# fanzhongyi/diffusion

Measured on AMD Instinct MI355X. Metric: U-Net training images/sec @256 (SD-2-base U-Net, precomputed latents 4x32x32), higher is better.
Workload: dtype bf16; 1 GPU; SD-2-base U-Net train step, latents 4x32x32, text 77x1024, batch 256/GPU (global 256), microbatch 256, AdamW, dp1; global_batch=256, microbatch=256, parallelism=dp1, params=865910724

## Files before the change

diffusion_amd/_lib.py:

```python
from __future__ import annotations

import ctypes as C
import os

_HERE = os.path.dirname(os.path.abspath(__file__))
LIB_PATH = os.path.join(_HERE, os.environ.get('DA_LIB_ALT') or 'libdiffusion_amd.so')

_vp, _l, _i, _f, _fp, _ll = C.c_void_p, C.c_long, C.c_int, C.c_float, C.c_void_p, C.c_void_p



class DaWgradItem(C.Structure):
    _fields_ = [('dY', C.c_void_p), ('lddy', C.c_long), ('X', C.c_void_p), ('ldx', C.c_long), ('dW', C.c_void_p),
                ('dbias', C.c_void_p), ('N', C.c_int), ('Cin', C.c_int)]


SIGNATURES = {
    'da_gemm_nt': [_vp, _l, _vp, _vp, _l, _fp, _vp, _l, _vp, _l, _i, _i, _i, _i, _i, _i, _i, _i, _i, _i, _i, _f, _fp, _l,
                   _vp],
    'da_set_option': [C.c_char_p, _i],
    'da_gemm_nt_variant_for': [_i, _i, _i, _i, _l],
    'da_gemm_nt_geglu': [_vp, _l, _vp, _vp, _l, _vp, _l, _fp, _i, _i, _i, _vp],
    'da_gemm_nt_geglu_bwd': [_vp, _l, _vp, _vp, _l, _vp, _l, _i, _i, _i, _vp],
    'da_gemm_tn_wgrad': [_vp, _l, _vp, _l, _fp, _fp, _fp, _i, _i, _i, _i, _i, _i, _i, _i, _i, _fp, _l, _vp],
    'da_gemm_tn_variant_for': [_i, _i, _i, _i, _i, _i, _i, _i, _i],
    'da_gemm_tn_wgrad_group': [C.POINTER(DaWgradItem), _i, _i, _fp, _l, _vp],
    'da_gemm_tn_group_plan': [C.POINTER(DaWgradItem), _i, _i, _l, C.POINTER(_i), _i, C.POINTER(_i)],
    'da_attn_fwd': [_vp, _l, _vp, _l, _vp, _l, _vp, _l, _fp, _i, _i, _i, _i, _f, _vp],
    'da_attn_fwd_causal': [_vp, _l, _vp, _l, _vp, _l, _vp, _l, _fp, _i, _i, _i, _f, _vp],
    'da_attn_fwd_wide': [_vp, _l, _vp, _l, _vp, _l, _vp, _l, _fp, _i, _i, _i, _i, _i, _f, _vp],
    'da_attn_bwd': [_vp, _l, _vp, _l, _vp, _l, _vp, _l, _vp, _l, _fp, _fp, _vp, _l, _vp, _l, _vp, _l, _i, _i, _i, _i,
                    _f, _vp],
    'da_norm_scratch_floats': [_i, _i, _i],
    'da_groupnorm_fwd': [_vp, _l, _vp, _l, _fp, _fp, _fp, _fp, _fp, _i, _i, _i, _i, _f, _i, _vp],
# ... 87 lines not shown
```

diffusion_amd/csrc/gemm_nt.hip:

```cpp
#include <string.h>

#include "common.hpp"
#include "diffusion_amd.h"

namespace {

struct GemmNTParams {
  const bf16* A;
  const bf16* W;
  void* C;
  const float* bias;
  const bf16* rowbias;
  const bf16* R;
  long lda, ldc, ldrb, ldr;
  int M, N, K, Cin;
  int Hin, Win, Hout, Wout;
  int ksize, mode;
  int out_fp32;
  float alpha;
  int tiles_m, tiles_n;
};

constexpr int BM = 128, BN = 128, BK = 64;
constexpr int STAGE_BYTES = (BM + BN) * BK * 2;
// ... 203 lines not shown
                           hipStream_t stream);

int da_gemm_nt_v3_try(const void* A, long lda, const void* W, void* C, long ldc, const float* bias, const void* R, long ldr,
                      int M, int N, int K, hipStream_t stream);
extern int g_nt_stream, g_nt_stream_lw;
int da_gemm_nt_ws_try(const void* A, long lda, const void* W, const float* bias, const void* R, long ldr, void* C, long ldc,
                      int M, int N, int K, hipStream_t stream);
extern int g_nt_ws;

extern int g_tn_variant;
extern int g_nt_korder;
extern int g_nt_persist;
extern int g_reserve_cus;
extern int g_nt_persist_conv;
extern int g_nt_de;
extern int g_grad_overwrite;
extern int g_attn_fused_bwd;
extern int g_tn_ring, g_tn_ungroup;
extern int g_gn_resident, g_gn_resident_form, g_gn_resident_min_slab;
int da_usable_cus(int cus);
static int g_nt_variant = 0;
static int g_nt_mfma32 = 0;
static int g_nt_splitk = 1;

static int g_nt_dispatch = 1;

static int pick_nt_variant_legacy(int M, int N, int K, int Cin, long ws_floats, int* splits) {
  *splits = 1;
  const long tm = (M + 255) / 256;
  if (N % 320 == 0 && tm * (N / 320) >= 160) return 12;
// ... 102 lines not shown
    return DA_OK;
  }
  if (key && !strcmp(key, "gemm_nt_stream_lw")) {
    if (value != 4 && value != 16) return DA_ERR_SHAPE;
    g_nt_stream_lw = value;
    return DA_OK;
  }
  if (key && !strcmp(key, "gemm_nt_stream")) {
    g_nt_stream = value;
    return DA_OK;
  }
  if (key && !strcmp(key, "gemm_nt_de")) {
    g_nt_de = value;
    return DA_OK;
  }
  if (key && !strcmp(key, "gemm_nt_persist_conv")) {
    g_nt_persist_conv = value;
    return DA_OK;
  }
  if (key && !strcmp(key, "gn_resident")) {
    if (value < 0) return DA_ERR_SHAPE;
    g_gn_resident = value;
    return DA_OK;
  }
  if (key && !strcmp(key, "gn_resident_min_slab")) {
    if (value < 0) return DA_ERR_SHAPE;
    g_gn_resident_min_slab = value;
    return DA_OK;
  }
  if (key && !strcmp(key, "gn_resident_form")) {
// ... 62 lines not shown
```

diffusion_amd/csrc/gemm_nt_v2.hip:

```cpp
#include "common.hpp"
#include "diffusion_amd.h"
#ifndef NT2_NT
#define NT2_NT 0
#endif
#if NT2_NT
#define NTST st8_nt
#else
#define NTST st8
#endif


#ifndef NT2_CT
#define NT2_CT 1
#endif

int g_nt_persist = -1;
int g_reserve_cus = 0;
int g_nt_persist_conv = 1;
int g_nt_de = 1;
int da_usable_cus(int cus) {
  int n = cus - g_reserve_cus;
  return n < 32 ? 32 : n;
}

// ... 12 lines not shown
  int ksize, mode;
  int out_fp32;
  float alpha;
  int tiles_m, tiles_n;
  int splits, ksteps_per_split;
  long slab_stride;
  bf16* G;
  long ldg;
  int inner;
  int total_blocks;
  FastDiv div_hw, div_w;
  FastDiv div_nblk, div_tn;
  int korder;
};

__device__ __attribute__((aligned(256))) unsigned char g_zero_page[256];

template <int BK>
DEVINL int swz_key(int row) { return BK == 64 ? ((row >> 1) & 7) : ((row >> 2) & 3); }
template <int BK>
DEVINL int swz2(int row, int chunk) { return row * (BK * 2) + ((chunk ^ swz_key<BK>(row)) << 4); }

DEVINL void lds_barrier() {
  asm volatile("s_waitcnt lgkmcnt(0)" ::: "memory");
  __builtin_amdgcn_s_barrier();
  asm volatile("" ::: "memory");
}

#ifdef DA_STAMPS
__device__ unsigned long long* g_stamp_buf;
// ... 2 lines not shown
    if (threadIdx.x == 0 && g_stamp_buf) g_stamp_buf[(long)vblock * 16 + (i)] = __builtin_amdgcn_s_memtime(); \
  } while (0)
extern "C" int da_debug_set_stamps(void* buf) {
  return hipMemcpyToSymbol(HIP_SYMBOL(g_stamp_buf), &buf, sizeof(buf)) == hipSuccess ? 0 : -1;
}
#else
#define STAMP(i) do {} while (0)
#endif

DEVINL void glds16(const void* gsrc, char* lds_dst) {
  __builtin_amdgcn_global_load_lds((const __attribute__((address_space(1))) void*)gsrc,
                                   (__attribute__((address_space(3))) void*)lds_dst, 16, 0, 0);
}

template <int MT, int NT, int WM, int WN, int BK, bool UPS, int GEGLU, bool EARLY, int MF = 16, bool PERSIST = EARLY, bool DE = false,
          bool HASR = false>
DEVINL void nt2_tile(const GemmNT2Params& p, const int vblock0, char* smem) {
  constexpr int NW = WM * WN;
  constexpr bool CT = MF == 16 && GEGLU == 0 && ((NT2_CT && !EARLY) || DE);
  static_assert(!DE || (MF == 16 && GEGLU == 0 && ((NT % 2) == 0 || (MT % 2) == 0)), "direct epilogue: 16x16 tiles in pairs");
  constexpr int V2_BM = MF * MT * WM, V2_BK = BK;
  static_assert((NW == 16 || NW == 8 || NW == 4) && (BK == 64 || BK == 32), "wave grid");
  static_assert(MF == 16 || (MF == 32 && GEGLU == 0 && BK == 64), "MFMA shape");
  constexpr int BN = MF * NT * WN;
  constexpr int SR = MF == 16 ? 16 : 8;
  constexpr int RG = 512 / BK;
  constexpr int LR = BK / 8;
  constexpr int AJ = V2_BM / RG / NW;
  constexpr int BGROUPS = BN / RG;
  constexpr int BJ = (BGROUPS + NW - 1) / NW;
  constexpr int A_BYTES = V2_BM * V2_BK * 2;
  constexpr int B_BYTES = BN * V2_BK * 2;
// ... 11 lines not shown
  auto task_of = [&](int ln, int pss, int tasks) {
    const bool ragged_last = (tasks % (64 * WN)) != 0 && pss == (tasks + 64 * WN - 1) / (64 * WN) - 1;
    const int slot = ragged_last ? (wn + WN - (wm * WN / 4) % WN) % WN : wn;
    return slot * 64 + ln + 64 * WN * pss;
  };
  auto fresh_lane = [&]() {
    int ln = lane;
    asm volatile("" : "+v"(ln));
    return ln;
  };
  STAMP(0);

  const int nblk = p.tiles_m * p.tiles_n;
  int split, tn, m0, n0;
  auto locate = [&](int vb) {
    split = (PERSIST && !EARLY) ? (int)fdiv((unsigned)vb, p.div_nblk) : vb / nblk;
    int bid = vb - split * nblk;
    const int q = nblk >> 3, r = nblk & 7;
    const int xcd = bid & 7, idx = bid >> 3;
    bid = (xcd < r ? xcd * (q + 1) : r * (q + 1) + (xcd - r) * q) + idx;
    const int tm = (PERSIST && !EARLY) ? (int)fdiv((unsigned)bid, p.div_tn) : bid / p.tiles_n;
    tn = bid - tm * p.tiles_n;
    m0 = tm * V2_BM;
    n0 = tn * BN;
  };
  auto wrow = [&](int c) {
    if constexpr (GEGLU == 1) return c < BN / 2 ? tn * (BN / 2) + c : p.inner + tn * (BN / 2) + (c - BN / 2);
    else return n0 + c;
  };
  const int HWo = p.Hout * p.Wout;
  constexpr bool PCONV = PERSIST && !EARLY;
  const int pad = PCONV ? 1 : ((p.ksize == 3 && p.mode != 4) ? 1 : 0);
  const int gmul = PCONV ? 1 : ((p.mode == 1 || p.mode == 4) ? 2 : 1), gshift = PCONV ? 0 : ((p.mode == 2 || p.mode == 3) ? 1 : 0),
            pmask = PCONV ? 0 : ((p.mode == 2) ? 1 : 0);
  const int hlim = gshift ? 2 * p.Hin : p.Hin, wlim = gshift ? 2 * p.Win : p.Win;
  const char* zero = reinterpret_cast<const char*>(g_zero_page);
  auto load_bias = [&](int buf) {
    if (tid < BN / 4) {
      const int n = wrow(tid * 4);
      const void* src = (p.bias && n < p.N) ? (const void*)(p.bias + n) : (const void*)zero;
      glds16(src, smem + BIAS_OFF + buf * (BN * 4) + wave * 1024);
    }
  };

  const int ntaps = PCONV ? 9 : p.ksize * p.ksize;
  const bf16* abase[AJ];
  unsigned amask[AJ];
  unsigned aoff[AJ];
  unsigned woff[BJ];
  int nk, tap, c0;
  const int nk_total = p.K / V2_BK;
  const bool tap_inner = p.korder != 0 && ntaps > 1;
  auto describe = [&]() {
  const int dl = fresh_lane();
  const int lrow = dl / LR, lchunk = dl % LR;
#pragma unroll
// ... 30 lines not shown
    }
    const int bh = (oh * gmul - pad) >> gshift, bw = (ow * gmul - pad) >> gshift;
    if constexpr (PERSIST && !UPS) {
      aoff[j] = (unsigned)(((long)(b * p.Hin * p.Win) + (long)bh * p.Win + bw) * p.lda * 2 + (lchunk ^ swz_key<BK>(row)) * 16);
      if (j == 0) amask[0] = mask & 0x1ffu;
      else amask[0] |= (mask & 0x1ffu) << (9 * j);
      continue;
    }
    amask[j] = mask;
    abase[j] = p.A + ((long)(b * p.Hin * p.Win) + (long)bh * p.Win + bw) * p.lda + (lchunk ^ swz_key<BK>(row)) * 8;
  }
#pragma unroll
  for (int j = 0; j < BJ; ++j) {
    const int g = wave + NW * j;
    const int row = g * RG + lrow;
    const int n = min(wrow(row), p.N - 1);
    woff[j] = ((unsigned)n * (unsigned)p.K + (lchunk ^ swz_key<BK>(row)) * 8) * 2;
  }

  const int kstep_begin = split * p.ksteps_per_split;
  nk = min(p.ksteps_per_split, nk_total - kstep_begin);
  if (tap_inner) {
    const int ch = kstep_begin / ntaps;
    tap = kstep_begin - ch * ntaps;
    c0 = ch * V2_BK;
  } else {
    const int kb = kstep_begin * V2_BK;
    tap = kb / p.Cin;
    c0 = kb - tap * p.Cin;
  }
  };
  auto issue = [&](int stage, bool live) {
// ... 22 lines not shown
        for (int j = 0; j < AJ; ++j) {
          const void* src = (amask[j] & tapbit) ? (const void*)(abase[j] + soff) : (const void*)zero;
          glds16(src, Ab + (wave * AJ + j) * 1024);
        }
      }
    } else {
#pragma unroll
      for (int j = 0; j < AJ; ++j) {
        const int ph = (amask[j] >> 16) & 1, pw = (amask[j] >> 17) & 1;
        const int dr = (r + pad * (1 - ph)) >> 1, ds = (s2 + pad * (1 - pw)) >> 1;
        const long soff = (long)(dr * p.Win + ds) * p.lda + c0;
        const void* src = (amask[j] & tapbit) ? (const void*)(abase[j] + soff) : (const void*)zero;
        glds16(src, Ab + (wave * AJ + j) * 1024);
      }
    }
    const char* wb = reinterpret_cast<const char*>(p.W + (live ? tap * p.Cin + c0 : 0));
#pragma unroll
    for (int j = 0; j < BJ; ++j) {
      const int g = wave + NW * j;
      if constexpr (PERSIST && !EARLY) {
        if (BGROUPS % NW == 0 || g < BGROUPS) glds16(wb + (size_t)j * (NW * RG) * p.K * 2 + woff[0], Bb + g * 1024);
      } else {
        if (BGROUPS % NW == 0 || g < BGROUPS) glds16(wb + woff[j], Bb + g * 1024);
      }
    }
    const int tap_n = tap + 1, c_n = c0 + V2_BK;
    const bool wrap_t = tap_n >= ntaps, wrap_c = c_n >= p.Cin;
    if (tap_inner) {
      tap = wrap_t ? 0 : tap_n;
      c0 = wrap_t ? c_n : c0;
    } else {
// ... 317 lines not shown

  constexpr bool EPI_DB = !PERSIST && 2 * WM * STRIP * 4 <= 2 * STAGE;
  constexpr int CH = BN / 8;
  constexpr int TASKS = SR * CH;
  constexpr int NSI = MT * (MF == 16 ? 1 : 4);
  constexpr int PASSES = (TASKS + 64 * WN - 1) / (64 * WN);
  constexpr int RBUD = NW == 16 ? 3 : 10;
  constexpr int RD = (NSI < RBUD / PASSES) ? NSI : (RBUD / PASSES < 1 ? 1 : RBUD / PASSES);
  int trow[PASSES], tcol[PASSES];
  bool tval[PASSES];
#pragma unroll
  for (int pss = 0; pss < PASSES; ++pss) {
    const int task = task_of(el, pss, TASKS);
    trow[pss] = task / CH;
    tcol[pss] = (task - trow[pss] * CH) * 8;
    tval[pss] = task < TASKS && n0e + tcol[pss] < p.N;
  }
  const int mrow0 = m0e + wm * (MF * MT);
  const bool has_r = p.R != nullptr && p.splits == 1;
  bf16x8 rres[RD][PASSES];
  auto fetch_r = [&](int i, int slot) {
#pragma unroll
    for (int pss = 0; pss < PASSES; ++pss) {
      const int m = mrow0 + i * SR + trow[pss];
      if (tval[pss] && m < p.M) rres[slot][pss] = ld8(p.R + (long)m * p.ldr + n0e + tcol[pss]);
    }
  };
#pragma unroll
  for (int i = 0; i < RD; ++i) {
#pragma unroll
// ... 53 lines not shown
          for (int e = 0; e < 8; ++e) v[e] += bf2f(rbv[e]);
        }
        if (has_r) {
          const bf16x8 rv = rres[i % RD][pss];
#pragma unroll
          for (int e = 0; e < 8; ++e) v[e] += bf2f(rv[e]);
        }
        if (p.out_fp32) {
          float* cp = reinterpret_cast<float*>(p.C) + (long)m * p.ldc + n;
          *reinterpret_cast<f32x4*>(cp) = f32x4{v[0], v[1], v[2], v[3]};
          *reinterpret_cast<f32x4*>(cp + 4) = f32x4{v[4], v[5], v[6], v[7]};
        } else {
          bf16x8 o;
#pragma unroll
          for (int e = 0; e < 8; ++e) o[e] = f2bf(v[e]);
          if constexpr (EARLY) NTST(reinterpret_cast<bf16*>(p.C) + (long)m * p.ldc + n, o);
          else st8(reinterpret_cast<bf16*>(p.C) + (long)m * p.ldc + n, o);
        }
      }
    }
    if (has_r && i + RD < NSI) fetch_r(i + RD, i % RD);
    if (!EPI_DB) lds_barrier();
    STAMP(4 + i);
  }
  };

  locate(vblock);
  load_bias(0);
  describe();
  issue(0, true);
  if constexpr (!PERSIST) {
    kloop(0);
    epilogue(m0, n0, tn, split, 0);
  } else {
    for (int bbuf = 0;; bbuf ^= 1) {
      kloop(bbuf);
      const int m0e = m0, n0e = n0, tne = tn, splite = split;
      const int vnext = vblock + (int)gridDim.x;
      const bool more = vnext < p.total_blocks;
      if (more) {
        locate(vnext);
        load_bias(bbuf ^ 1);
        describe();
        issue(0, true);
      }
      STAMP(8);
      epilogue(m0e, n0e, tne, splite, bbuf);
      STAMP(12);
      if (!more) break;
      vblock = vnext;
    }
  }
}

template <int MT, int NT, int WM, int WN, int BK, bool UPS, int GEGLU = 0, bool EARLY = false, int MF = 16, bool PERSIST = EARLY, bool DE = false,
          bool HASR = false>
__global__ __launch_bounds__(64 * WM * WN, (WM * WN == 16 ? 4 : 2)) void gemm_nt2_kernel(GemmNT2Params p) {
  extern __shared__ __attribute__((aligned(16))) char smem[];
  nt2_tile<MT, NT, WM, WN, BK, UPS, GEGLU, EARLY, MF, PERSIST, DE, HASR>(p, blockIdx.x, smem);
}

__global__ void splitk_finalize_kernel(GemmNT2Params p, const float* ws) {
  const int nvec = p.N >> 3;
  const long total = (long)p.M * nvec;
  const int HWo = p.Hout * p.Wout;
  for (long i = (long)blockIdx.x * blockDim.x + threadIdx.x; i < total; i += (long)gridDim.x * blockDim.x) {
    const long m = i / nvec;
    const int n = (int)(i - m * nvec) * 8;
    float v[8] = {0.f, 0.f, 0.f, 0.f, 0.f, 0.f, 0.f, 0.f};
#pragma unroll 4
    for (int s = 0; s < p.splits; ++s) {
      const float* src = ws + s * p.slab_stride + m * p.N + n;
      const f32x4 a = *reinterpret_cast<const f32x4*>(src), b = *reinterpret_cast<const f32x4*>(src + 4);
#pragma unroll
// ... 129 lines not shown
    if (p.ksize == 1 && (long)p.M * p.lda * 2 < (1L << 32)) return launch_v2_mode<MT, NT, WM, WN, BK, false, true, MF>(p, splits, ws, stream);
  }
  if constexpr (WM * WN == 16 && MF == 16 && MT == 4 && NT == 5) {
    const long tiles = (long)((p.M + 255) / 256) * ((p.N + 319) / 320) * (splits > 1 ? splits : 1);
    if (g_nt_persist_conv && g_nt_persist != 0 && p.ksize == 3 && p.mode == 0 && tiles > da_usable_cus(256) && p.N % 320 == 0 &&
        p.M < (1 << 24) && (long)p.M * p.Hout * p.Wout < (1L << 40) &&
        (long)(p.M / (p.Hout * p.Wout)) * p.Hin * p.Win * p.lda * 2 < (1L << 32))
      return launch_v2_mode<MT, NT, WM, WN, BK, false, false, MF, true>(p, splits, ws, stream);
  }
  return launch_v2_mode<MT, NT, WM, WN, BK, false, false, MF>(p, splits, ws, stream);
}

}

int g_nt_korder = 1;

int da_gemm_nt_v2_dispatch(int variant, int splits, float* ws, const void* A, long lda, const void* W, void* C, long ldc, const float* bias,
                           const void* rowbias, long ldrb, const void* R, long ldr, int M, int N, int K, int Cin,
                           int Hin, int Win, int Hout, int Wout, int ksize, int mode, int out_fp32, float alpha,
                           hipStream_t stream) {
  GemmNT2Params p;
  p.A = (const bf16*)A; p.W = (const bf16*)W; p.C = C; p.bias = bias;
  p.rowbias = (const bf16*)rowbias; p.R = (const bf16*)R;
  p.lda = lda; p.ldc = ldc; p.ldrb = ldrb; p.ldr = ldr;
  p.M = M; p.N = N; p.K = K; p.Cin = Cin;
  p.Hin = Hin; p.Win = Win; p.Hout = Hout; p.Wout = Wout;
  p.ksize = ksize; p.mode = mode; p.out_fp32 = out_fp32; p.alpha = alpha;
  p.tiles_m = p.tiles_n = 0;
  p.splits = 1; p.ksteps_per_split = 0; p.slab_stride = 0;
  p.G = nullptr; p.ldg = 0; p.inner = 0;
// ... 62 lines not shown
```

diffusion_amd/models/unet.py:

```python
from __future__ import annotations

import math
import os
from dataclasses import dataclass
from typing import Dict, List, Optional, Tuple

import torch
import torch.nn as nn

from .. import ops
from ..ops import BF16, F32, Geom


@dataclass
class UNetConfig:
    in_channels: int = 4
    out_channels: int = 4
    block_out_channels: Tuple[int, ...] = (320, 640, 1280, 1280)
    attention_head_dim: Tuple[int, ...] = (5, 10, 20, 20)
    cross_attention_dim: int = 1024
    layers_per_block: int = 2
    norm_num_groups: int = 32
    norm_eps: float = 1e-5
    sample_size: int = 64
# ... 286 lines not shown
        self.exp_avg_sq = torch.zeros(fp.total, device=dev, dtype=F32)
        self.shadow = torch.zeros(fp.total, device=dev, dtype=BF16)
        self.shadow_t = torch.zeros(max(fp.total_t, 8), device=dev, dtype=BF16)
        self._bind_views()
        self._scratch = None
        self._scratch_key = None
        self.opt_step = 0
        self._grad_fresh = False
        self._grad_ready_cb = None
        import os
        self.wgrad_stream = torch.cuda.Stream() if os.environ.get('DA_WGRAD_STREAM', '0') == '1' else None
        self._wgrad_defer = None
        self._tape = None
        self._kv, self._record = None, True
        self._ctx = self._tproj = None
        if init:
            self.reset_parameters(seed)

    def _bind_views(self):
        fp = self.fp
        self._mats: Dict[str, Mat] = {}
        self._vecs: Dict[str, Vec] = {}
        for name, st in fp.storages.items():
            sl = slice(st.off, st.off + st.numel)
            if st.ntc is not None:
                N, T, C = st.ntc
                m = Mat()
                m.N, m.T, m.C = N, T, C
                m.w = self.shadow[sl].view(N, T * C)
                m.gw = self.grad[sl].view(N, T * C)
# ... 266 lines not shown
        tb = p + '.transformer_blocks.0'
        g, gst = self._gn_fwd(x, p + '.norm', B, HW, 1e-6, 0)
        h0 = self._lin_fwd(g, p + '.proj_in')
        n1, ln1 = self._ln_fwd(h0, tb + '.norm1')
        qkv = self._bf(M, 3 * C)
        ops.gemm_nt(n1, self.M(tb + '.attn1.qkv.weight').w, qkv, Geom.linear(M))
        o1 = self._bf(M, C)
        l1 = self._f32(B * heads * HW)
        ops.attn_fwd(qkv[:, :C], qkv[:, C:2 * C], qkv[:, 2 * C:], o1, l1, B, heads, HW, HW, 0.125)
        h1 = self._lin_fwd(o1, tb + '.attn1.to_out.0', residual=h0)
        n2, ln2 = self._ln_fwd(h1, tb + '.norm2')
        q2 = self._lin_fwd(n2, tb + '.attn2.to_q', bias=False)
        nk = self._ctx.shape[0] // B
        if self._kv is not None:
            kv2 = self._kv[p]
        else:
            kv2 = self._bf(B * nk, 2 * C)
            ops.gemm_nt(self._ctx, self.M(tb + '.attn2.kv.weight').w, kv2, Geom.linear(B * nk))
        o2 = self._bf(M, C)
        l2 = self._f32(B * heads * HW)
        ops.attn_fwd(q2, kv2[:, :C], kv2[:, C:], o2, l2, B, heads, HW, nk, 0.125)
        h2 = self._lin_fwd(o2, tb + '.attn2.to_out.0', residual=h1)
        n3, ln3 = self._ln_fwd(h2, tb + '.norm3')
        gg = self._bf(M, 4 * C)
        if ops.geglu_fusable(4 * C, C):
            f = self._bf(M, 8 * C)
            ops.gemm_nt_geglu(n3, self.M(tb + '.ff.net.0.proj.weight').w, f, gg, self.V(tb + '.ff.net.0.proj.bias').p)
        else:
            f = self._lin_fwd(n3, tb + '.ff.net.0.proj')
            ops.geglu_fwd(f, gg)
# ... 26 lines not shown
        if ops.geglu_bwd_fusable(4 * C, C):
            self._lin_bwd(gg, dh3, tb + '.ff.net.2', need_dx=False)
            ops.gemm_nt_geglu_bwd(dh3, self.M(tb + '.ff.net.2.weight').wt, f, df)
        else:
            dgg = self._lin_bwd(gg, dh3, tb + '.ff.net.2')
            ops.geglu_bwd(f, dgg, df)
            del dgg
        dn3 = self._lin_bwd(n3, df, tb + '.ff.net.0.proj')
        del df
        dh2 = self._ln_bwd(h2, dn3, dh3, tb + '.norm3', ln3)
        do2 = self._lin_bwd(o2, dh2, tb + '.attn2.to_out.0')
        dq2 = self._bf(M, C)
        dkv2 = self._bf(B * nk, 2 * C)
        ops.attn_bwd(q2, kv2[:, :C], kv2[:, C:], o2, do2, l2, self._delta, dq2, dkv2[:, :C], dkv2[:, C:], B, heads, HW,
                     nk, 0.125)
        self._wgrad(dkv2, self._ctx, self.M(tb + '.attn2.kv.weight').gw, Geom.linear(B * nk))
        dn2 = self._lin_bwd(n2, dq2, tb + '.attn2.to_q', bias=False)
        dh1 = self._ln_bwd(h1, dn2, dh2, tb + '.norm2', ln2)
        do1 = self._lin_bwd(o1, dh1, tb + '.attn1.to_out.0')
        dqkv = self._bf(M, 3 * C)
        ops.attn_bwd(qkv[:, :C], qkv[:, C:2 * C], qkv[:, 2 * C:], o1, do1, l1, self._delta, dqkv[:, :C],
                     dqkv[:, C:2 * C], dqkv[:, 2 * C:], B, heads, HW, HW, 0.125)
        mq = self.M(tb + '.attn1.qkv.weight')
        self._wgrad(dqkv, n1, mq.gw, Geom.linear(M))
        dn1 = self._bf(M, C)
        ops.gemm_nt(dqkv, mq.wt, dn1, Geom.linear(M))
        dh0 = self._ln_bwd(h0, dn1, dh1, tb + '.norm1', ln1)
        dg = self._lin_bwd(g, dh0, p + '.proj_in')
        if self._wgrad_defer is not None:
            items, self._wgrad_defer = self._wgrad_defer[1], None
            ops.gemm_tn_wgrad_group(items, M)
# ... 3 lines not shown
    def forward_features(self, xt8: torch.Tensor, t: torch.Tensor, ctx: torch.Tensor, B: int, S, kv=None,
                         record: bool = True):
        if kv is None and record:
            return self._walk(xt8, t, ctx, B, S)
        if kv is not None and record:
            raise ValueError('forward_features: kv is for the forward-only walk (backward needs the projections it made)')
        keep = (self._ctx, self._tproj)
        self._kv, self._record = kv, False
        try:
            return self._walk(xt8, t, ctx, B, S)
        finally:
            self._kv, self._record = None, True
            self._ctx, self._tproj = keep

    def project_context(self, ctx: torch.Tensor):
        kv = {}
        for key in self._mats:
            if key.endswith('.attn2.kv.weight'):
                m = self.M(key)
                out = self._bf(ctx.shape[0], m.N)
                ops.gemm_nt(ctx, m.w, out, Geom.linear(ctx.shape[0]))
                kv[key[:-len('.transformer_blocks.0.attn2.kv.weight')]] = out
        return kv

    def _walk(self, xt8, t, ctx, B, S):
        cfg = self.cfg
        boc = cfg.block_out_channels
        n = len(boc)
        record = self._record
        H, W = spatial_hw(S)
        self.check_spatial(H, W)
        if xt8.shape[0] != B * H * W:
            raise ValueError(f'forward_features: {xt8.shape[0]} input rows for B * H * W = {B} * {H} * {W}')
        self._ensure_scratch(B, H, W)
        self._ctx = ctx
        tape = [] if record else _NoTape()
        te0 = self._bf(B, boc[0])
        if t.dtype == F32:
            ops.timestep_embed_f32(t, te0)
        else:
            ops.timestep_embed(t, te0)
        te1 = self._lin_fwd(te0, 'time_embedding.linear_1')
        te1s = self._bf(B, cfg.time_embed_dim)
        ops.silu_fwd(te1, te1s)
        temb = self._lin_fwd(te1s, 'time_embedding.linear_2')
        tembs = self._bf(B, cfg.time_embed_dim)
        ops.silu_fwd(temb, tembs)
        self._tproj = self._bf(B, self.tproj_total)
        ops.gemm_nt(tembs, self.M('time_emb_proj_all.weight').w, self._tproj, Geom.linear(B),
                    bias=self.V('time_emb_proj_all.bias').p)
# ... 65 lines not shown
                    tape.append(('resnet', sv))
                    h, sv = self._transformer_fwd(f'up_blocks.{i}.attentions.{j}', h, B, rh, rw, rev_heads[i], out=nxt)
                    tape.append(('transformer', sv))
                else:
                    h, sv = self._resnet_fwd(p, cat, B, rh, rw, out=nxt)
                    tape.append(('resnet', sv))
                if not record:
                    cats[s] = cat = None
                s -= 1
            if i < n - 1:
                key = f'up_blocks.{i}.upsamplers.0.conv'
                y = cats[s][:, :cat_cb[s]]
                ops.gemm_nt(h, self.M(key + '.weight').w, y, Geom.up(B, rh, rw), bias=self.V(key + '.bias').p)
                tape.append(('up', (key, h, B, rh, rw)))
                h = y
        a, st = self._gn_fwd(h, 'conv_norm_out', B, H * W, cfg.norm_eps, 1)
        pred = torch.empty(B * H * W, 8, device=self.device_, dtype=F32)
        ops.gemm_nt(a, self.M('conv_out.weight').w, pred, Geom.conv(B, H, W), bias=self.V('conv_out.bias').p)
        if not record:
            return pred
        tape.append(('out', (h, a, st, B, H, W)))
        self._tape = tape
        self._cats = cats
        return pred

    def backward_features(self, dpred: torch.Tensor):
        tape, self._tape = self._tape, None
        if tape is None:
            raise RuntimeError('backward_features called without a recorded forward')
        fresh, self._grad_fresh = getattr(self, '_grad_fresh', False), False
        if fresh:
            ops.set_option('grad_overwrite', 1)
        try:
            self._backward_walk(tape, dpred)
        finally:
            if fresh:
                ops.set_option('grad_overwrite', 0)

    def _backward_walk(self, tape, dpred: torch.Tensor):
        B = dpred.shape[0]
        self._dtproj = self._bf(self._tproj.shape[0], self.tproj_total)
        dskip: Dict[int, torch.Tensor] = {}
        dh = None
        off = lambda name: self.fp.storages[name].off
        for kind, sv in reversed(tape):
            lo = None
            if kind == 'out':
                lo = off('conv_norm_out.weight')
                h, a, st, B, H, W = sv
                m = self.M('conv_out.weight')
                g3 = Geom.conv(B, H, W)
                self._wgrad(dpred, a, m.gw, g3, dbias=self.V('conv_out.bias').g, scratch=self._scratch)
                da = self._bf(B * H * W, m.C)
                ops.gemm_nt(dpred, m.wt, da, g3)
                dh = self._gn_bwd(h, da, None, 'conv_norm_out', st, B, H * W, 1)
            elif kind == 'resnet':
                dh = self._resnet_bwd(sv, dh)
                lo = off(sv[0] + '.norm1.weight')
            elif kind == 'transformer':
# ... 27 lines not shown
                ops.gemm_nt(dh, m.wt, dx, Geom.down_dgrad(B, rh, rw))
                dh = dx
            elif kind == 'conv_in':
                xt8, B, H, W = sv
                tot = self._bf(*dh.shape)
                ops.add(dh, dskip.pop(0), tot)
                self._wgrad(tot, xt8, self.M('conv_in.weight').gw, Geom.conv(B, H, W),
                                  dbias=self.V('conv_in.bias').g, scratch=self._scratch)
                lo = off('conv_in.weight')
            else:
                raise AssertionError(kind)
            if lo is not None and self._grad_ready_cb is not None:
                if self.wgrad_stream is not None:
                    torch.cuda.current_stream().wait_stream(self.wgrad_stream)
                self._grad_ready_cb(lo)
        te0, te1, te1s, temb, tembs = self._temb_saved
        Bt = te0.shape[0]
        mt = self.M('time_emb_proj_all.weight')
        self._wgrad(self._dtproj, tembs, mt.gw, Geom.linear(Bt), dbias=self.V('time_emb_proj_all.bias').g,
                          scratch=self._scratch)
        dtembs = self._bf(Bt, mt.C)
        ops.gemm_nt(self._dtproj, mt.wt, dtembs, Geom.linear(Bt))
        dtemb = self._bf(Bt, mt.C)
        ops.silu_bwd(temb, dtembs, dtemb)
        dte1s = self._lin_bwd(te1s, dtemb, 'time_embedding.linear_2')
        dte1 = self._bf(*te1.shape)
        ops.silu_bwd(te1, dte1s, dte1)
        self._lin_bwd(te0, dte1, 'time_embedding.linear_1', need_dx=False)
        if self.wgrad_stream is not None:
            torch.cuda.current_stream().wait_stream(self.wgrad_stream)
# ... 32 lines not shown
```

diffusion_amd/ops.py:

```python
from __future__ import annotations

import ctypes
import os
from typing import Optional, Tuple

import torch

from . import _lib

BF16 = torch.bfloat16
F32 = torch.float32


def _stream() -> int:
    return torch.cuda.current_stream().cuda_stream


SPLITK_WS = None


PROFILE = None


class _Timed:
# ... 122 lines not shown
                14: 'gemm_nt2_kernel<4,4,4,4>', 15: 'gemm_nt2_kernel<1,5,8,2,mf32>', 16: 'gemm_nt2_kernel<2,5,4,2,mf32>',
                18: 'gemm_nt2_kernel<3,4,8,2>'}[v]
        ws = _opt('gemm_nt_ws', 1)
        ws_bn = 320 if (K == 320 and (ws & 1) and N <= 1280) else 128 if (K == 640 and (ws & 2) and N <= 1024) else 0
        if (ws_bn and _opt('gemm_nt_variant', 0) == 0 and N % ws_bn == 0 and M % 32 == 0 and (M // 32) * (N // ws_bn) >= 8 * 256
                and g.ksize == 1 and g.mode == 0 and not out_fp32 and alpha == 1.0 and rowbias is None):
            name = 'gemm_nt_ws_kernel'
    with _Timed(name, flops, (M, N, K, g.ksize, g.mode)):
        _lib.call('da_gemm_nt', a_ptr, lda, w_ptr, c_ptr, ldc, _vec(bias, N, 'bias'), rb_ptr, ldrb, r_ptr, ldr, M, N,
                  K, Cin, g.Hin, g.Win, g.Hout, g.Wout, g.ksize, g.mode, int(out_fp32), float(alpha),
                  SPLITK_WS.data_ptr() if SPLITK_WS is not None else 0,
                  SPLITK_WS.numel() if SPLITK_WS is not None else 0, _stream())
    return out


def geglu_fusable(inner: int, K: int) -> bool:
    return inner % 160 == 0 and K % 64 == 0


def gemm_nt_geglu(A, W, F, G, bias):
    a_ptr, lda = _mat(A, BF16, 'A')
    w_ptr, ldw = _mat(W, BF16, 'W')
    f_ptr, ldf = _mat(F, BF16, 'F')
    g_ptr, ldg = _mat(G, BF16, 'G')
    M, K = A.shape
    inner = G.shape[1]
    if tuple(W.shape) != (2 * inner, K) or ldw != K or tuple(F.shape) != (M, 2 * inner) or G.shape[0] != M:
        raise ValueError('gemm_nt_geglu: shape mismatch')
    if not geglu_fusable(inner, K):
        raise ValueError(f'gemm_nt_geglu needs inner % 160 == 0 and K % 64 == 0, got {inner}, {K}')
# ... 660 lines not shown
```

include/diffusion_amd.h:

```cpp
#ifndef DIFFUSION_AMD_H
#define DIFFUSION_AMD_H

#ifdef __cplusplus
extern "C" {
#endif

typedef struct ihipStream_t* da_stream_t;

int da_gemm_nt(const void* A, long lda, const void* W, void* C, long ldc, const float* bias, const void* rowbias,
               long ldrb, const void* R, long ldr, int M, int N, int K, int Cin, int Hin, int Win, int Hout, int Wout,
               int ksize, int mode, int out_fp32, float alpha, float* splitk_ws, long splitk_ws_floats,
               da_stream_t stream);

int da_gemm_nt_geglu(const void* A, long lda, const void* W, void* F, long ldf, void* G, long ldg, const float* bias,
                     int M, int inner, int K, da_stream_t stream);

int da_gemm_nt_geglu_bwd(const void* dY, long lddy, const void* Wt, const void* F, long ldf, void* dF, long lddf, int M,
                         int inner, int K, da_stream_t stream);

int da_set_option(const char* key, int value);
int da_gemm_nt_variant_for(int M, int N, int K, int Cin, long splitk_ws_floats);

int da_gemm_tn_wgrad(const void* dY, long lddy, const void* X, long ldx, float* dW, float* dbias, float* scratch, int M,
                     int N, int Cin, int Hin, int Win, int Hout, int Wout, int ksize, int mode, float* split_ws,
                     long split_ws_floats, da_stream_t stream);

int da_gemm_tn_variant_for(int M, int N, int Cin, int Hin, int Win, int Hout, int Wout, int ksize, int mode);

typedef struct DaWgradItem {
  const void* dY;
  long lddy;
  const void* X;
  long ldx;
// ... 148 lines not shown
```

Before: 1586 images/sec.

## Group cross-attention KV projections into one persistent GEMM and batch their wgrads

Adds a grouped persistent GEMM kernel that computes every cross-attention KV projection of the shared text context in a single launch (up to 16 weight matrices). Tiles are walked in patches across the concatenated N dimension. The forward pass precomputes all KV projections up front, and the backward pass defers the KV weight-gradient GEMMs into one grouped wgrad call at the end. This cuts many small launches and under-filled GEMMs on the 77-token context. The cost is holding all KV outputs live across the whole forward pass, plus a new, complex tile-mapping code path.

```diff
diff --git a/diffusion_amd/_lib.py b/diffusion_amd/_lib.py
--- a/diffusion_amd/_lib.py
+++ b/diffusion_amd/_lib.py
@@ -15,9 +15,16 @@
                 ('dbias', C.c_void_p), ('N', C.c_int), ('Cin', C.c_int)]
 
 
+class DaGemmNtItem(C.Structure):
+    _fields_ = [('W', C.c_void_p), ('C', C.c_void_p), ('ldc', C.c_long), ('bias', C.c_void_p), ('N', C.c_int),
+                ('reserved', C.c_int)]
+
+
 SIGNATURES = {
     'da_gemm_nt': [_vp, _l, _vp, _vp, _l, _fp, _vp, _l, _vp, _l, _i, _i, _i, _i, _i, _i, _i, _i, _i, _i, _i, _f, _fp, _l,
                    _vp],
+    'da_gemm_nt_group': [_vp, _l, C.POINTER(DaGemmNtItem), _i, _i, _i, _vp],
+    'da_gemm_nt_group_plan': [C.POINTER(DaGemmNtItem), _i, _i, _i],
     'da_set_option': [C.c_char_p, _i],
     'da_gemm_nt_variant_for': [_i, _i, _i, _i, _l],
     'da_gemm_nt_geglu': [_vp, _l, _vp, _vp, _l, _vp, _l, _fp, _i, _i, _i, _vp],
diff --git a/diffusion_amd/csrc/gemm_nt.hip b/diffusion_amd/csrc/gemm_nt.hip
--- a/diffusion_amd/csrc/gemm_nt.hip
+++ b/diffusion_amd/csrc/gemm_nt.hip
@@ -241,6 +241,7 @@
 extern int g_reserve_cus;
 extern int g_nt_persist_conv;
 extern int g_nt_de;
+extern int g_kv_group, g_nt_group_patch;
 extern int g_grad_overwrite;
 extern int g_attn_fused_bwd;
 extern int g_tn_ring, g_tn_ungroup;
@@ -373,6 +374,16 @@
     g_nt_de = value;
     return DA_OK;
   }
+  if (key && !strcmp(key, "kv_group")) {
+    if (value != 0 && value != 1) return DA_ERR_SHAPE;
+    g_kv_group = value;
+    return DA_OK;
+  }
+  if (key && !strcmp(key, "gemm_nt_group_patch")) {
+    if (value < 0 || value > 9999) return DA_ERR_SHAPE;
+    g_nt_group_patch = value;
+    return DA_OK;
+  }
   if (key && !strcmp(key, "gemm_nt_persist_conv")) {
     g_nt_persist_conv = value;
     return DA_OK;
diff --git a/diffusion_amd/csrc/gemm_nt_v2.hip b/diffusion_amd/csrc/gemm_nt_v2.hip
--- a/diffusion_amd/csrc/gemm_nt_v2.hip
+++ b/diffusion_amd/csrc/gemm_nt_v2.hip
@@ -50,6 +50,27 @@
   int korder;
 };
 
+constexpr int NT_GROUP_MAX = 16;
+struct NtGroupItem {
+  const bf16* W;
+  bf16* C;
+  const float* bias;
+  long ldc;
+  int N;
+  int first;
+};
+struct NtGroupParams {
+  NtGroupItem it[NT_GROUP_MAX];
+  int patch_m, patch_n;
+};
+
+struct NtGroupState {
+  int item, eitem;
+  const bf16* W;
+  const float* bias;
+  int N;
+};
+
 __device__ __attribute__((aligned(256))) unsigned char g_zero_page[256];
 
 template <int BK>
@@ -82,8 +103,9 @@
 }
 
 template <int MT, int NT, int WM, int WN, int BK, bool UPS, int GEGLU, bool EARLY, int MF = 16, bool PERSIST = EARLY, bool DE = false,
-          bool HASR = false>
-DEVINL void nt2_tile(const GemmNT2Params& p, const int vblock0, char* smem) {
+          bool HASR = false, bool GROUP = false>
+DEVINL void nt2_tile(const GemmNT2Params& p, const int vblock0, char* smem, const NtGroupParams* gp = nullptr, NtGroupState* gs = nullptr) {
+  static_assert(!GROUP || (EARLY && PERSIST && GEGLU == 0 && !DE && !HASR && !UPS && MF == 16), "grouped form: persistent linear tile walk");
   constexpr int NW = WM * WN;
   constexpr bool CT = MF == 16 && GEGLU == 0 && ((NT2_CT && !EARLY) || DE);
   static_assert(!DE || (MF == 16 && GEGLU == 0 && ((NT % 2) == 0 || (MT % 2) == 0)), "direct epilogue: 16x16 tiles in pairs");
@@ -125,6 +147,34 @@
   const int nblk = p.tiles_m * p.tiles_n;
   int split, tn, m0, n0;
   auto locate = [&](int vb) {
+    if constexpr (GROUP) {
+      const int nb = p.tiles_m * p.tiles_n;
+      const int q = nb >> 3, r = nb & 7;
+      const int xcd = vb & 7, idx = vb >> 3;
+      const int bid = (xcd < r ? xcd * (q + 1) : r * (q + 1) + (xcd - r) * q) + idx;
+      const int band_tiles = p.tiles_m * gp->patch_n;
+      const int cb = min(bid / band_tiles, (p.tiles_n - 1) / gp->patch_n);
+      const int bb = bid - cb * band_tiles;
+      const int w = min(gp->patch_n, p.tiles_n - cb * gp->patch_n);
+      const int pt = gp->patch_m * w;
+      const int rp = bb / pt, rem = bb - rp * pt;
+      const int pr = rem / w;
+      const int tm = rp * gp->patch_m + pr, tc = cb * gp->patch_n + (rem - pr * w);
+      int it = 0;
+#pragma unroll
+      for (int i = 1; i < NT_GROUP_MAX; ++i)
+        if (tc >= gp->it[i].first) it = i;
+      it = __builtin_amdgcn_readfirstlane(it);
+      gs->item = it;
+      gs->W = gp->it[it].W;
+      gs->bias = gp->it[it].bias;
+      gs->N = gp->it[it].N;
+      split = 0;
+      tn = tc - gp->it[it].first;
+      m0 = tm * V2_BM;
+      n0 = tn * BN;
+      return;
+    }
     split = (PERSIST && !EARLY) ? (int)fdiv((unsigned)vb, p.div_nblk) : vb / nblk;
     int bid = vb - split * nblk;
     const int q = nblk >> 3, r = nblk & 7;
@@ -149,8 +199,13 @@
   auto load_bias = [&](int buf) {
     if (tid < BN / 4) {
       const int n = wrow(tid * 4);
+      if constexpr (GROUP) {
+        const void* src = (gs->bias && n < gs->N) ? (const void*)(gs->bias + n) : (const void*)zero;
+        glds16(src, smem + BIAS_OFF + buf * (BN * 4) + wave * 1024);
+      } else {
       const void* src = (p.bias && n < p.N) ? (const void*)(p.bias + n) : (const void*)zero;
       glds16(src, smem + BIAS_OFF + buf * (BN * 4) + wave * 1024);
+      }
     }
   };
 
@@ -211,8 +266,13 @@
   for (int j = 0; j < BJ; ++j) {
     const int g = wave + NW * j;
     const int row = g * RG + lrow;
+    if constexpr (GROUP) {
+      const int n = min(wrow(row), gs->N - 1);
+      woff[j] = ((unsigned)n * (unsigned)p.K + (lchunk ^ swz_key<BK>(row)) * 8) * 2;
+    } else {
     const int n = min(wrow(row), p.N - 1);
     woff[j] = ((unsigned)n * (unsigned)p.K + (lchunk ^ swz_key<BK>(row)) * 8) * 2;
+    }
   }
 
   const int kstep_begin = split * p.ksteps_per_split;
@@ -265,7 +325,9 @@
         glds16(src, Ab + (wave * AJ + j) * 1024);
       }
     }
-    const char* wb = reinterpret_cast<const char*>(p.W + (live ? tap * p.Cin + c0 : 0));
+    const char* wb;
+    if constexpr (GROUP) wb = reinterpret_cast<const char*>(gs->W + (live ? c0 : 0));
+    else wb = reinterpret_cast<const char*>(p.W + (live ? tap * p.Cin + c0 : 0));
 #pragma unroll
     for (int j = 0; j < BJ; ++j) {
       const int g = wave + NW * j;
@@ -613,6 +675,8 @@
     const int task = task_of(el, pss, TASKS);
     trow[pss] = task / CH;
     tcol[pss] = (task - trow[pss] * CH) * 8;
+    if constexpr (GROUP) tval[pss] = task < TASKS && n0e + tcol[pss] < gp->it[gs->eitem].N;
+    else
     tval[pss] = task < TASKS && n0e + tcol[pss] < p.N;
   }
   const int mrow0 = m0e + wm * (MF * MT);
@@ -696,6 +760,8 @@
           bf16x8 o;
 #pragma unroll
           for (int e = 0; e < 8; ++e) o[e] = f2bf(v[e]);
+          if constexpr (GROUP) NTST(gp->it[gs->eitem].C + (long)m * gp->it[gs->eitem].ldc + n, o);
+          else
           if constexpr (EARLY) NTST(reinterpret_cast<bf16*>(p.C) + (long)m * p.ldc + n, o);
           else st8(reinterpret_cast<bf16*>(p.C) + (long)m * p.ldc + n, o);
         }
@@ -718,6 +784,7 @@
     for (int bbuf = 0;; bbuf ^= 1) {
       kloop(bbuf);
       const int m0e = m0, n0e = n0, tne = tn, splite = split;
+      if constexpr (GROUP) gs->eitem = gs->item;
       const int vnext = vblock + (int)gridDim.x;
       const bool more = vnext < p.total_blocks;
       if (more) {
@@ -740,6 +807,12 @@
 __global__ __launch_bounds__(64 * WM * WN, (WM * WN == 16 ? 4 : 2)) void gemm_nt2_kernel(GemmNT2Params p) {
   extern __shared__ __attribute__((aligned(16))) char smem[];
   nt2_tile<MT, NT, WM, WN, BK, UPS, GEGLU, EARLY, MF, PERSIST, DE, HASR>(p, blockIdx.x, smem);
+}
+
+__global__ __launch_bounds__(1024, 4) void gemm_nt2_group_kernel(GemmNT2Params p, NtGroupParams g) {
+  extern __shared__ __attribute__((aligned(16))) char smem[];
+  NtGroupState st;
+  nt2_tile<4, 5, 4, 4, 64, false, 0, true, 16, true, false, false, true>(p, blockIdx.x, smem, &g, &st);
 }
 
 __global__ void splitk_finalize_kernel(GemmNT2Params p, const float* ws) {
@@ -899,6 +972,88 @@
 }
 
 int g_nt_korder = 1;
+int g_kv_group = 1;
+int g_nt_group_patch = 0;
+
+namespace {
+
+constexpr int NTG_PATCH_M = 6, NTG_PATCH_N = 6;
+
+int ntg_validate(const void* A, long lda, const DaGemmNtItem* items, int n_items, int M, int K, bool pointers) {
+  if (n_items < 0 || (n_items > 0 && !items) || M <= 0 || K <= 0) return DA_ERR_SHAPE;
+  if ((K % 64) || (lda & 7) || lda < K) return DA_ERR_SHAPE;
+  if ((long)M * lda * 2 >= (1L << 32)) return DA_ERR_SHAPE;
+  if (pointers && (!A || ((uintptr_t)A & 15))) return DA_ERR_SHAPE;
+  for (int i = 0; i < n_items; ++i) {
+    const DaGemmNtItem& it = items[i];
+    if (it.N <= 0 || (it.N & 7) || (it.ldc & 7) || it.ldc < it.N) return DA_ERR_SHAPE;
+    if ((long)it.N * K * 2 >= (1L << 32)) return DA_ERR_SHAPE;
+    if (pointers && (!it.W || !it.C || ((uintptr_t)it.W & 15) || ((uintptr_t)it.C & 15))) return DA_ERR_SHAPE;
+  }
+  return DA_OK;
+}
+
+int ntg_launch(const void* A, long lda, const DaGemmNtItem* items, int n, int M, int K, hipStream_t stream) {
+  constexpr int BN = 320, STAGE = 256 * 64 * 2 + BN * 64 * 2, STRIPS = 4 * 16 * (BN + 4) * 4;
+  constexpr int SMEM = (STAGE + STRIPS > 2 * STAGE ? STAGE + STRIPS : 2 * STAGE) + 2 * BN * 4;
+  static_assert(SMEM <= 160 * 1024, "LDS");
+  GemmNT2Params p;
+  NtGroupParams g;
+  int first = 0;
+  for (int i = 0; i < NT_GROUP_MAX; ++i) {
+    const DaGemmNtItem& it = items[i < n ? i : 0];
+    g.it[i].W = (const bf16*)it.W; g.it[i].C = (bf16*)it.C; g.it[i].bias = it.bias; g.it[i].ldc = it.ldc; g.it[i].N = it.N;
+    g.it[i].first = i < n ? first : 0x7fffffff;
+    if (i < n) first += (it.N + BN - 1) / BN;
+  }
+  const int pm = g_nt_group_patch / 100, pn = g_nt_group_patch % 100;
+  g.patch_m = pm > 0 ? pm : NTG_PATCH_M;
+  g.patch_n = pn > 0 ? pn : NTG_PATCH_N;
+  p.A = (const bf16*)A; p.W = g.it[0].W; p.C = g.it[0].C; p.bias = nullptr;
+  p.rowbias = nullptr; p.R = nullptr;
+  p.lda = lda; p.ldc = g.it[0].ldc; p.ldrb = 0; p.ldr = 0;
+  p.M = M; p.N = g.it[0].N; p.K = K; p.Cin = K;
+  p.Hin = 1; p.Win = 1; p.Hout = 1; p.Wout = 1;
+  p.ksize = 1; p.mode = 0; p.out_fp32 = 0; p.alpha = 1.0f;
+  p.tiles_m = (M + 255) / 256;
+  p.tiles_n = first;
+  p.splits = 1; p.ksteps_per_split = K / 64; p.slab_stride = 0;
+  p.G = nullptr; p.ldg = 0; p.inner = 0; p.korder = 0;
+  p.div_hw = p.div_w = p.div_nblk = p.div_tn = make_fastdiv(1u);
+  if ((long)p.tiles_m * p.tiles_n >= (1L << 20)) return DA_ERR_SHAPE;
+  p.total_blocks = p.tiles_m * p.tiles_n;
+  static unsigned long long attr_done = 0;
+  if (da_ensure_dyn_smem((const void*)gemm_nt2_group_kernel, SMEM, &attr_done) != DA_OK) return DA_ERR_LAUNCH;
+  hipLaunchKernelGGL(gemm_nt2_group_kernel, dim3(persistent_grid(p.total_blocks)), dim3(1024), SMEM, stream, p, g);
+  DA_CHECK_LAUNCH();
+  return DA_OK;
+}
+
+}
+
+extern "C" int da_gemm_nt_group_plan(const DaGemmNtItem* items, int n_items, int M, int K) {
+  if (ntg_validate(nullptr, K, items, n_items, M, K, false) != DA_OK) return -1;
+  return g_kv_group ? (n_items + NT_GROUP_MAX - 1) / NT_GROUP_MAX : 0;
+}
+
+extern "C" int da_gemm_nt_group(const void* A, long lda, const DaGemmNtItem* items, int n_items, int M, int K, hipStream_t stream) {
+  DA_CLEAR_ERR();
+  if (ntg_validate(A, lda, items, n_items, M, K, true) != DA_OK) return DA_ERR_SHAPE;
+  if (!g_kv_group) {
+    for (int i = 0; i < n_items; ++i) {
+      const int rc = da_gemm_nt(A, lda, items[i].W, items[i].C, items[i].ldc, items[i].bias, nullptr, 0, nullptr, 0, M, items[i].N, K, K, 1, 1,
+                                1, 1, 1, 0, 0, 1.0f, nullptr, 0, stream);
+      if (rc != DA_OK) return rc;
+    }
+    return DA_OK;
+  }
+  for (int base = 0; base < n_items; base += NT_GROUP_MAX) {
+    const int n = n_items - base < NT_GROUP_MAX ? n_items - base : NT_GROUP_MAX;
+    const int rc = ntg_launch(A, lda, items + base, n, M, K, stream);
+    if (rc != DA_OK) return rc;
+  }
+  return DA_OK;
+}
 
 int da_gemm_nt_v2_dispatch(int variant, int splits, float* ws, const void* A, long lda, const void* W, void* C, long ldc, const float* bias,
                            const void* rowbias, long ldrb, const void* R, long ldr, int M, int N, int K, int Cin,
diff --git a/diffusion_amd/models/unet.py b/diffusion_amd/models/unet.py
--- a/diffusion_amd/models/unet.py
+++ b/diffusion_amd/models/unet.py
@@ -324,6 +324,8 @@
         self._tape = None
         self._kv, self._record = None, True
         self._ctx = self._tproj = None
+        self._kv_walk = None
+        self._kv_wgrads = None
         if init:
             self.reset_parameters(seed)
 
@@ -620,6 +622,8 @@
         nk = self._ctx.shape[0] // B
         if self._kv is not None:
             kv2 = self._kv[p]
+        elif self._kv_walk is not None:
+            kv2 = self._kv_walk.pop(p)
         else:
             kv2 = self._bf(B * nk, 2 * C)
             ops.gemm_nt(self._ctx, self.M(tb + '.attn2.kv.weight').w, kv2, Geom.linear(B * nk))
@@ -676,7 +680,10 @@
         dkv2 = self._bf(B * nk, 2 * C)
         ops.attn_bwd(q2, kv2[:, :C], kv2[:, C:], o2, do2, l2, self._delta, dq2, dkv2[:, :C], dkv2[:, C:], B, heads, HW,
                      nk, 0.125)
-        self._wgrad(dkv2, self._ctx, self.M(tb + '.attn2.kv.weight').gw, Geom.linear(B * nk))
+        if self._kv_wgrads is not None:
+            self._kv_wgrads.append((dkv2, self._ctx, self.M(tb + '.attn2.kv.weight').gw, None))
+        else:
+            self._wgrad(dkv2, self._ctx, self.M(tb + '.attn2.kv.weight').gw, Geom.linear(B * nk))
         dn2 = self._lin_bwd(n2, dq2, tb + '.attn2.to_q', bias=False)
         dh1 = self._ln_bwd(h1, dn2, dh2, tb + '.norm2', ln2)
         do1 = self._lin_bwd(o1, dh1, tb + '.attn1.to_out.0')
@@ -710,13 +717,18 @@
             self._ctx, self._tproj = keep
 
     def project_context(self, ctx: torch.Tensor):
-        kv = {}
+        kv, items = {}, []
+        grouped = ops.kv_group() and ctx.shape[1] % 64 == 0
         for key in self._mats:
             if key.endswith('.attn2.kv.weight'):
                 m = self.M(key)
                 out = self._bf(ctx.shape[0], m.N)
-                ops.gemm_nt(ctx, m.w, out, Geom.linear(ctx.shape[0]))
+                if grouped:
+                    items.append((m.w, out, None))
+                else:
+                    ops.gemm_nt(ctx, m.w, out, Geom.linear(ctx.shape[0]))
                 kv[key[:-len('.transformer_blocks.0.attn2.kv.weight')]] = out
+        ops.gemm_nt_group(ctx, items)
         return kv
 
     def _walk(self, xt8, t, ctx, B, S):
@@ -730,6 +742,9 @@
             raise ValueError(f'forward_features: {xt8.shape[0]} input rows for B * H * W = {B} * {H} * {W}')
         self._ensure_scratch(B, H, W)
         self._ctx = ctx
+        self._kv_walk = None
+        if self._kv is None and ops.kv_group() and ctx.shape[1] % 64 == 0:
+            self._kv_walk = self.project_context(ctx)
         tape = [] if record else _NoTape()
         te0 = self._bf(B, boc[0])
         if t.dtype == F32:
@@ -825,6 +840,7 @@
                 ops.gemm_nt(h, self.M(key + '.weight').w, y, Geom.up(B, rh, rw), bias=self.V(key + '.bias').p)
                 tape.append(('up', (key, h, B, rh, rw)))
                 h = y
+        self._kv_walk = None
         a, st = self._gn_fwd(h, 'conv_norm_out', B, H * W, cfg.norm_eps, 1)
         pred = torch.empty(B * H * W, 8, device=self.device_, dtype=F32)
         ops.gemm_nt(a, self.M('conv_out.weight').w, pred, Geom.conv(B, H, W), bias=self.V('conv_out.bias').p)
@@ -854,6 +870,16 @@
         dskip: Dict[int, torch.Tensor] = {}
         dh = None
         off = lambda name: self.fp.storages[name].off
+        self._kv_wgrads = [] if (ops.kv_group() and self._grad_ready_cb is None and self.wgrad_stream is None) else None
+        try:
+            self._backward_tape(tape, dpred, dskip, dh, off)
+            if self._kv_wgrads:
+                ops.gemm_tn_wgrad_group(self._kv_wgrads, self._ctx.shape[0])
+        finally:
+            self._kv_wgrads = None
+        self._backward_time_path()
+
+    def _backward_tape(self, tape, dpred, dskip, dh, off):
         for kind, sv in reversed(tape):
             lo = None
             if kind == 'out':
@@ -911,6 +937,8 @@
                 if self.wgrad_stream is not None:
                     torch.cuda.current_stream().wait_stream(self.wgrad_stream)
                 self._grad_ready_cb(lo)
+
+    def _backward_time_path(self):
         te0, te1, te1s, temb, tembs = self._temb_saved
         Bt = te0.shape[0]
         mt = self.M('time_emb_proj_all.weight')
diff --git a/diffusion_amd/ops.py b/diffusion_amd/ops.py
--- a/diffusion_amd/ops.py
+++ b/diffusion_amd/ops.py
@@ -160,6 +160,47 @@
     return out
 
 
+def kv_group() -> bool:
+    return _opt('kv_group', 1) != 0
+
+
+def _nt_items(A, items):
+    M, K = A.shape
+    arr = (_lib.DaGemmNtItem * max(len(items), 1))()
+    flops = 0.0
+    for i, (W, out, bias) in enumerate(items):
+        w_ptr, ldw = _mat(W, BF16, f'items[{i}].W')
+        N = W.shape[0]
+        if ldw != K or W.shape[1] != K:
+            raise ValueError(f'items[{i}].W must be contiguous [N, {K}], got {tuple(W.shape)} ld {ldw}')
+        c_ptr, ldc = _mat(out, BF16, f'items[{i}].out')
+        if tuple(out.shape) != (M, N):
+            raise ValueError(f'items[{i}].out shape {tuple(out.shape)} != {(M, N)}')
+        arr[i] = _lib.DaGemmNtItem(w_ptr, c_ptr, ldc, _vec(bias, N, f'items[{i}].bias') or None, N, 0)
+        flops += 2.0 * M * N * K
+    return arr, flops
+
+
+def gemm_nt_group(A, items):
+    if not items:
+        return
+    a_ptr, lda = _mat(A, BF16, 'A')
+    M, K = A.shape
+    arr, flops = _nt_items(A, items)
+    with _Timed('gemm_nt_group', flops, (M, len(items), K, 1, 'group')):
+        _lib.call('da_gemm_nt_group', a_ptr, lda, arr, len(items), M, K, _stream())
+
+
+def gemm_nt_group_plan(Ns, M, K) -> int:
+    arr = (_lib.DaGemmNtItem * max(len(Ns), 1))()
+    for i, N in enumerate(Ns):
+        arr[i] = _lib.DaGemmNtItem(None, None, N, None, N, 0)
+    n = _lib.load().da_gemm_nt_group_plan(arr, len(Ns), M, K)
+    if n < 0:
+        raise ValueError('da_gemm_nt_group_plan rejected the arguments')
+    return n
+
+
 def geglu_fusable(inner: int, K: int) -> bool:
     return inner % 160 == 0 and K % 64 == 0
 
diff --git a/include/diffusion_amd.h b/include/diffusion_amd.h
--- a/include/diffusion_amd.h
+++ b/include/diffusion_amd.h
@@ -17,6 +17,18 @@
 
 int da_gemm_nt_geglu_bwd(const void* dY, long lddy, const void* Wt, const void* F, long ldf, void* dF, long lddf, int M,
                          int inner, int K, da_stream_t stream);
+
+typedef struct DaGemmNtItem {
+  const void* W;
+  void* C;
+  long ldc;
+  const float* bias;
+  int N;
+  int reserved;
+} DaGemmNtItem;
+
+int da_gemm_nt_group(const void* A, long lda, const DaGemmNtItem* items, int n_items, int M, int K, da_stream_t stream);
+int da_gemm_nt_group_plan(const DaGemmNtItem* items, int n_items, int M, int K);
 
 int da_set_option(const char* key, int value);
 int da_gemm_nt_variant_for(int M, int N, int K, int Cin, long splitk_ws_floats);
```

New measurement: 1590 images/sec (median of 6 runs). No clear change (+0.3%).
